# jantonguirao/nvImageCodec

Measured on AMD Instinct MI355X. Metric: images/sec, batched 1920x1080 4:2:0 baseline JPEG decode to interleaved RGB u8, higher is better.
Workload: dtype int32

## Files before the change

### nvimagecodec_amd/csrc/gpu_huffman.hip

```cpp
#include <hip/hip_runtime.h>

#include "gpu_huffman.h"
#include "huffman_gpu_core.h"

namespace hipjpeg {

namespace {

constexpr int kThreads = 256;

constexpr int kRowShift = kSubseqWords == 32 ? 5 : kSubseqWords == 16 ? 4 : kSubseqWords == 64 ? 6 : -1;
static_assert(kRowShift > 0, "subsequences of 512, 1024 or 2048 bits");

#define HJ_LDS __attribute__((address_space(3)))
#define HJ_GLOBAL __attribute__((address_space(1)))
typedef unsigned int u32x4 __attribute__((ext_vector_type(4)));

struct KSlot {
    int16_t* base;
    uint32_t stride_y, stride_x;
};

constexpr int kStagedExtra = 2;
constexpr int kRowWords = kSubseqWords + kStagedExtra;
// ... 312 lines not shown
    const bool markers = im.restart_interval != 0;
    uint32_t before = 0;
    for (uint32_t c = t; c < u.first; c += kThreads) before += drops[im.first_chunk + c];
    before = wg_sum(before, scratch);
    const uint32_t chunk_begin = u.first * kDestuffChunk;
    const uint32_t chunk_len = min((uint32_t)kDestuffChunk, raw_bytes - chunk_begin);
    const uint32_t gout = chunk_begin - before;
    const uint32_t a = gout & 3;

    {
        const uint32_t pieces = (chunk_len + 15) / 16;
        const HJ_GLOBAL u32x4* src = (const HJ_GLOBAL u32x4*)(im.raw + chunk_begin);
        constexpr uint32_t kPiecesPerLane = kDestuffChunk / 16 / kThreads;
        u32x4 v[kPiecesPerLane];
#pragma unroll
        for (uint32_t i = 0; i < kPiecesPerLane; i++) v[i] = src[min(i * kThreads + t, pieces - 1)];
#pragma unroll
        for (uint32_t i = 0; i < kPiecesPerLane; i++) {
            const uint32_t q = i * kThreads + t, g = q * 4 + (q >> 2);
            const u32x4 x = q < pieces ? v[i] : u32x4{0x01010101u, 0x01010101u, 0x01010101u, 0x01010101u};
            buf[g] = x.x;
            buf[g + 1] = x.y;
            buf[g + 2] = x.z;
            buf[g + 3] = x.w;
        }
    }
    const uint32_t before_chunk = chunk_begin > 0 ? im.raw[chunk_begin - 1] : 0u;
    const uint32_t behind_chunk = chunk_len == (uint32_t)kDestuffChunk ? im.raw[chunk_begin + kDestuffChunk] : 0x01u;
    __syncthreads();

    const uint32_t off = chunk_begin + t * 64;
    uint32_t x[16];
    uint32_t gone[4] = {0, 0, 0, 0};
    uint32_t n = 0, len = 0;
    if (off < raw_bytes) {
        len = min(64u, raw_bytes - off);
        const uint32_t pieces = (len + 15) / 16;
        const uint32_t before_lane = t > 0 ? buf[(t - 1) * 17 + 15] >> 24 : before_chunk;
#pragma unroll
        for (uint32_t i = 0; i < 16; i++) x[i] = i < pieces * 4 ? buf[t * 17 + i] : 0x01010101u;
        uint32_t d[16];
        uint32_t prev = before_lane;
#pragma unroll
        for (uint32_t i = 0; i < 16; i++) {
            d[i] = stuffed_zero_mask(x[i], prev);
            prev = x[i] >> 24;
        }
        if (markers) {
            const uint32_t behind = pieces == 4 ? (t < kThreads - 1 ? buf[(t + 1) * 17] & 0xFFu : behind_chunk) : 0x01u;
            prev = before_lane;
#pragma unroll
            for (uint32_t i = 0; i < 16; i++) {
                d[i] |= marker_mask(x[i], prev, i < 15 ? (x[i < 15 ? i + 1 : 15] & 0xFFu) : behind);
                prev = x[i] >> 24;
            }
        }
#pragma unroll
        for (uint32_t i = 0; i < 16; i++) {
            const uint32_t p = __popc(d[i]);
            n += p;
            gone[i / 5] |= p << (6 * (i % 5) + 3);
            const uint32_t m = __builtin_amdgcn_udot4(d[i], 0x08040201u, 0u, false) >> 7;
            x[i] = __builtin_amdgcn_perm(x[i], x[i], squeeze_sel[m]);
        }
    }
    uint32_t incl = n;
    for (int d = 1; d < 64; d <<= 1) {
        const uint32_t v = __shfl_up(incl, d);
        if ((t & 63) >= d) incl += v;
    }
    if ((t & 63) == 63) wave_base[t >> 6] = incl;
    __syncthreads();
    uint32_t excl = incl - n;
    for (int w = 0; w < (t >> 6); w++) excl += wave_base[w];
    const uint32_t chunk_drops = wave_base[0] + wave_base[1] + wave_base[2] + wave_base[3];
    auto padded = [](uint32_t k) { return k + ((k >> 6) << 2); };
    const uint32_t o0 = a + t * 64 - excl, cnt0 = o0 & 3;
    uint32_t slot = o0 >> 2, bits = 8 * cnt0, acc = 0;
    if (len) {
#pragma unroll
        for (uint32_t i = 0; i < 16; i++) {
            const unsigned long long w = (unsigned long long)x[i] << bits;
            const uint32_t p = (gone[i / 5] >> (6 * (i % 5))) & 63u;
            const bool full = bits >= p;
            acc |= (uint32_t)w;
            if (full) buf[slot + (slot >> 4)] = acc;
            acc = full ? (uint32_t)(w >> 32) : acc;
            slot += full ? 1u : 0u;
            bits = (bits - p) & 24u;
        }
    }
    const uint32_t o = slot * 4, cnt = bits / 8;
    __syncthreads();
    {
        const uint32_t from = slot == (o0 >> 2) ? cnt0 : 0u;
#pragma unroll
        for (uint32_t b = 0; b < 3; b++)
            if (b >= from && b < cnt) bytes[padded(o + b)] = (uint8_t)((uint32_t)acc >> (8 * b));
    }
    __syncthreads();
    const uint32_t n_out = chunk_len - chunk_drops;
    uint8_t* dst = const_cast<uint8_t*>(im.stream) + (gout - a);
    const uint32_t first_full = a ? 1 : 0, end_full = (a + n_out) / 4;
    for (uint32_t d = first_full + t; d < end_full; d += kThreads) reinterpret_cast<uint32_t*>(dst)[d] = buf[d + (d >> 4)];
    if (t < 4) {
        if (a && (uint32_t)t >= a && (uint32_t)t < a + n_out) dst[t] = bytes[padded((uint32_t)t)];
        const uint32_t tail = max(end_full, first_full) * 4 + t;
        if (tail >= a && tail < a + n_out && tail >= 4 * first_full) dst[tail] = bytes[padded(tail)];
    }
    if (chunk_begin + chunk_len == raw_bytes) {
        const uint32_t total = raw_bytes - before - chunk_drops;
        const uint32_t padded = ((total + 3) & ~3u) + kStreamSlackBytes;
        uint8_t* s = const_cast<uint8_t*>(im.stream);
        if (total + t < padded) s[total + t] = 0xFF;
        if (t == 0) {
            im.total_bits = total * 8;
            im.num_subseq = (total * 8 + kSubseqBits - 1) / kSubseqBits;
            im.stream_words = padded / 4;
        }
    }
}

__global__ __launch_bounds__(kSyncThreads) void huff_sync_kernel(const HuffImage* __restrict__ images, const HuffUnit* __restrict__ units,
                                                             unsigned long long* __restrict__ states, unsigned long long* __restrict__ incoming,
                                                             unsigned int* __restrict__ counters, int first_pass, int max_rounds,
                                                             uint16_t* __restrict__ tail_tasks, uint32_t* __restrict__ tail_count, uint16_t* records)
{
    __shared__ WgShared sh;
    extern __shared__ uint16_t dyn_pool[];
    HJ_LDS uint16_t* pool = (HJ_LDS uint16_t*)dyn_pool;
    const HuffUnit u = units[blockIdx.x];
    const HuffImage& im = images[u.image];
    const HuffGeom geom = make_geom(im);
    const uint32_t nsub = (geom.total_bits + kSubseqBits - 1) / kSubseqBits;
    if (u.first >= nsub) return;
    unsigned long long* gstate = states + im.first_subseq;
    const int t = threadIdx.x;
    const uint32_t j = u.first - 1 + t;
    const bool owner = t >= 1 && j < nsub;
    const int n_rows = (int)min((uint32_t)kSyncThreads, nsub - u.first + 1);
    unsigned long long in_state = 0;
    if (!first_pass) {
        in_state = u.first ? __hip_atomic_load(&gstate[u.first - 1], __ATOMIC_RELAXED, __HIP_MEMORY_SCOPE_AGENT) & kSyncMask : 0ull;
        if (in_state == incoming[blockIdx.x]) return;
    }
    stage_rows<kSyncThreads>(sh.stream, im, (int)u.first - 1);
    stage_pool<kSyncThreads>(pool, im);
    stage_constants(sh.tsel, nullptr, nullptr, im, false);
    __syncthreads();

    DevEnv env = make_env(sh, pool, u.first, geom);
    const bool rst = im.restart_interval != 0;
    unsigned long long old_global = ~0ull;
    int task = -1;
    const bool recording = !rst;
    if (first_pass) {
        const unsigned long long assumed = (unsigned long long)j * kSubseqBits;
        unsigned long long mine = 0;
        if (owner || (t == 0 && u.first > 0)) {
            const uint32_t bidx0 = boundary0_of(im, j);
            env.set_row(t);
            mine = pack_state(walk_subsequence(rst, false, geom, env, j * kSubseqBits, (j + 1) * kSubseqBits, 0, 0, bidx0, SlotRecorder()));
        }
        sh.end[t] = mine;
        __syncthreads();
        if (owner && ((sh.end[t - 1] & kSyncMask) != assumed || recording)) task = t;
    } else {
        if (owner) old_global = gstate[j];
        sh.end[t] = t == 0 ? in_state : old_global;
        if (t == 1) task = 1;
    }
    int rounds = 0;
    for (int round = 0; round < kSyncThreads + 2; round++) {
        __syncthreads();
        rounds++;
        unsigned long long now = 0;
        bool moved = false;
        if (task >= 0) {
            const SubseqState p = unpack_state(sh.end[task - 1]);
            env.set_row(task);
            const uint32_t jt = u.first - 1 + task;
            const SlotRecorder rec = slot_recorder(records, im, jt);
            const SubseqState st = walk_subsequence(rst, recording, geom, env, p.end_bit, (jt + 1) * kSubseqBits, p.zk & 255, p.zk >> 8, boundary0_of(im, jt), rec);
            if (recording) put_mark(rec, p.end_bit, (jt + 1) * kSubseqBits, geom.total_bits, p.zk & 255, st);
            now = pack_state(st);
            moved = ((now ^ sh.end[task]) & kSyncMask) != 0;
        }
        __syncthreads();
        if (task >= 0) sh.end[task] = now;
        const int pending = compact_tasks(sh, moved && task + 1 < n_rows, task + 1, &task);
        if (pending == 0 || rounds >= max_rounds) {
            if (tail_count) {
                if (t < pending) tail_tasks[(size_t)blockIdx.x * kSyncThreads + t] = (uint16_t)task;
                if (t == 0) tail_count[blockIdx.x] = (uint32_t)pending;
            }
            break;
        }
    }
    __syncthreads();
    if (owner) {
        const unsigned long long mine = sh.end[t];
        if (mine != old_global) {
            __hip_atomic_store(&gstate[j], mine, __ATOMIC_RELAXED, __HIP_MEMORY_SCOPE_AGENT);
            if (t == n_rows - 1 && ((mine ^ old_global) & kSyncMask) != 0) atomicAdd(counters + (first_pass ? 1 : 0), 1u);
        }
    }
    if (t == 0) {
        incoming[blockIdx.x] = first_pass ? (sh.end[0] & kSyncMask) : in_state;
        atomicAdd(counters + (first_pass ? 2 : 4), (unsigned)rounds);
        atomicMax(counters + (first_pass ? 3 : 5), (unsigned)rounds);
    }
}

constexpr int kTailWaves = 4;
constexpr int kTailThreads = 64 * kTailWaves;
#ifndef HJ_TAIL_SLOTS
#define HJ_TAIL_SLOTS 32
#endif
constexpr int kTailSlots = HJ_TAIL_SLOTS;
static_assert(kTailSlots == 32 || kTailSlots == 64, "a power of two, at most one row buffer per lane");
constexpr int kTailRowWords = kSubseqWords + 4;

struct TailWave {
    uint32_t rows[kTailSlots * kTailRowWords];
    uint16_t list[2][kSyncThreads];
    uint32_t count[2];
};
struct TailShared {
    TailWave wave[kTailWaves];
    uint32_t tsel[10];
};

struct TailEnv {
    uint32_t row_base;
    uint32_t word0;
    uint32_t pool;
    const HJ_LDS uint32_t* tsel;
    const uint32_t* boundaries;
    uint32_t num_boundaries;
    __device__ __forceinline__ uint32_t boundary(uint32_t i) const { return load_boundary(boundaries, num_boundaries, i); }
    static constexpr uint32_t kCursorStep = (uint32_t)kTailSlots * 4u;
    __device__ __forceinline__ uint32_t cursor(uint32_t i) const { return row_base + (i - word0) * kCursorStep; }
    __device__ __forceinline__ uint32_t fetch(uint32_t c) const { return *(const HJ_LDS uint32_t*)(uintptr_t)c; }
    __device__ __forceinline__ uint32_t tables(int k) const { return tsel[k]; }
    __device__ __forceinline__ uint32_t lookup1(uint32_t t, uint32_t w) const
    {
        return *(const HJ_LDS uint16_t*)(uintptr_t)(pool + t + ((w >> (31 - kHuffFastBits)) & ((2u << kHuffFastBits) - 2)));
    }
    __device__ __forceinline__ uint32_t lookup2(uint32_t e, uint32_t w) const
    {
        return *(const HJ_LDS uint16_t*)(uintptr_t)(pool + ((e & 0x1FFu) << 7) + ((w >> 15) & ((2u << kHuffSubBits) - 2)));
    }
    __device__ __forceinline__ uint32_t lookup_pair(uint32_t t, uint32_t w) const
    {
        return *(const HJ_LDS uint16_t*)(uintptr_t)(pool + t + 2 * kPairOffset + ((w >> (31 - kHuffFastBits)) & ((2u << kHuffFastBits) - 2)));
    }
};

__device__ __forceinline__ void wave_sync()
{
    __builtin_amdgcn_fence(__ATOMIC_ACQ_REL, "workgroup");
    __builtin_amdgcn_wave_barrier();
}


__device__ __forceinline__ unsigned long long state_in_front(const unsigned long long* states, const HuffImage& im, const HuffUnit u)
{
    return u.first ? __hip_atomic_load(&states[im.first_subseq + u.first - 1], __ATOMIC_RELAXED, __HIP_MEMORY_SCOPE_AGENT) & kSyncMask : 0ull;
}

__device__ __forceinline__ uint32_t uni(uint32_t v) { return (uint32_t)__builtin_amdgcn_readfirstlane((int)v); }
__device__ __forceinline__ uint32_t lane_read(uint32_t v, uint32_t lane) { return (uint32_t)__builtin_amdgcn_readlane((int)v, (int)lane); }

struct CoopWindow {
    uint32_t pool;
    const HJ_LDS uint32_t* tsel;
    const HJ_LDS uint32_t* row;
    uint32_t row_bit0, lane;
    uint32_t edc, eac;
    __device__ __forceinline__ uint32_t tables(uint32_t k) const { return tsel[k]; }
    __device__ __forceinline__ uint32_t entry(uint32_t table, uint32_t w) const
    {
        uint32_t e = *(const HJ_LDS uint16_t*)(uintptr_t)(pool + table + ((w >> (31 - kHuffFastBits)) & ((2u << kHuffFastBits) - 2)));
        if ((e >> 9) == kZadvLong) e = *(const HJ_LDS uint16_t*)(uintptr_t)(pool + ((e & 0x1FFu) << 7) + ((w >> 15) & ((2u << kHuffSubBits) - 2)));
        return e;
    }
    __device__ __forceinline__ void open(uint32_t pos, uint32_t ts)
    {
        const uint32_t b = pos + lane - row_bit0, bit = b & 31u;
        const uint32_t w0 = row[(b >> 5) * kTailSlots], w1 = row[((b >> 5) + 1) * kTailSlots];
        const uint32_t w = bit ? __builtin_amdgcn_alignbit(w0, w1, 32u - bit) : w0;
        edc = entry(ts & 0xFFFFu, w);
        eac = entry(ts >> 16, w);
    }
    __device__ __forceinline__ uint32_t dc(uint32_t rel) const { return lane_read(edc, rel); }
    __device__ __forceinline__ uint32_t ac(uint32_t rel) const { return lane_read(eac, rel); }
};

constexpr int kTailRoundBudget = 192, kRippleRoundBudget = 192;
#ifndef HJ_COOP_CHAINS
#define HJ_COOP_CHAINS 2
#endif
constexpr int kCoopChains = HJ_COOP_CHAINS;

template <bool RIPPLE>
__device__ __forceinline__ void tail_group(TailWave& ws, TailEnv env, HuffImage& im, const HuffUnit u, uint32_t ui, int lane,
                                           unsigned long long* __restrict__ states, unsigned long long* __restrict__ incoming,
                                           unsigned int* __restrict__ counters, const uint16_t* __restrict__ tail_tasks, uint32_t pending,
                                           uint32_t pass_id, uint16_t* records)
{
    const HuffGeom geom = make_geom(im);
    const uint32_t nsub = (geom.total_bits + kSubseqBits - 1) / kSubseqBits;
    if (u.first >= nsub) return;
    unsigned long long* gstate = states + im.first_subseq;
    const int n_rows = (int)min((uint32_t)kSyncThreads, nsub - u.first + 1);
    unsigned long long entering;
    if (RIPPLE) {
        entering = state_in_front(states, im, u);
        if (lane == 0) {
            incoming[ui] = entering;
            ws.list[0][0] = 1;
        }
    } else {
        entering = incoming[ui];
        for (uint32_t i = lane; i < pending; i += 64) ws.list[0][i] = tail_tasks[(size_t)ui * kSyncThreads + i];
    }
    if (lane == 0) ws.count[0] = pending;
    wave_sync();
    const bool rst = im.restart_interval != 0;
    const bool recording = !rst;
    bool out_moved = false;
    const HJ_GLOBAL uint32_t* g = (const HJ_GLOBAL uint32_t*)im.stream;
    const uint32_t gwords = im.stream_words;
    env.row_base = (uint32_t)(uintptr_t)(HJ_LDS uint32_t*)&ws.rows[lane & (kTailSlots - 1)];
    int rounds = 0, cur = 0;
    bool unfinished = false;
    for (int round = 0;; round++) {
        const uint32_t n = ws.count[cur];
        if (n == 0) break;
        if (round >= (RIPPLE ? kRippleRoundBudget : kTailRoundBudget)) {
            unfinished = true;
            break;
        }
        rounds++;
        wave_sync();
        if (lane == 0) ws.count[cur ^ 1] = 0;
        wave_sync();
        if (kCoopChains > 0 && n <= (uint32_t)kCoopChains && !rst) {
            CoopWindow win;
            win.pool = env.pool;
            win.tsel = env.tsel;
            win.row = (const HJ_LDS uint32_t*)&ws.rows[0];
            win.lane = (uint32_t)lane;
            win.edc = win.eac = 0;
            const uint32_t changes = cooperative_table_changes(win, geom.blocks_per_mcu);
            for (uint32_t q = 0; q < n && !unfinished; q++) {
                for (int task = (int)uni(ws.list[cur][q]);; task++) {
                    if (rounds++ >= (RIPPLE ? kRippleRoundBudget : kTailRoundBudget)) {
                        unfinished = true;
                        break;
                    }
                    const unsigned long long before =
                        task == 1 ? entering : __hip_atomic_load(&gstate[u.first - 2 + task], __ATOMIC_RELAXED, __HIP_MEMORY_SCOPE_AGENT);
                    const unsigned long long old = __hip_atomic_load(&gstate[u.first - 1 + task], __ATOMIC_RELAXED, __HIP_MEMORY_SCOPE_AGENT);
                    const uint32_t word0 = (u.first - 1 + task) * kSubseqWords;
                    wave_sync();
                    if (lane < kTailRowWords) {
                        const uint32_t d = word0 + lane;
                        ws.rows[lane * kTailSlots] = d < gwords ? __builtin_bswap32(g[d]) : ~0u;
                    }
                    wave_sync();
                    const SubseqState p = unpack_state(before);
                    win.row_bit0 = word0 * 32u;
                    const uint32_t jt = u.first - 1 + task;
                    const SlotRecorder rec = slot_recorder(records, im, jt);
                    const SubseqState st = cooperative_subsequence(geom, win, changes, p.end_bit, (jt + 1) * kSubseqBits, p.zk & 255u, p.zk >> 8, rec);
                    if (lane == 0) put_mark(rec, p.end_bit, (jt + 1) * kSubseqBits, geom.total_bits, p.zk & 255u, st);
                    const unsigned long long now = pack_state(st);
                    const bool moved = ((now ^ old) & kSyncMask) != 0;
                    if (lane == 0) __hip_atomic_store(&gstate[u.first - 1 + task], now, __ATOMIC_RELAXED, __HIP_MEMORY_SCOPE_AGENT);
                    wave_sync();
                    if (!moved) break;
                    if (task + 1 >= n_rows) {
                        out_moved = true;
                        break;
                    }
                }
            }
            break;
        }
        for (uint32_t base = 0; base < n; base += kTailSlots) {
            const bool busy = lane < kTailSlots && base + lane < n;
            const int task = busy ? (int)ws.list[cur][base + lane] : 1;
            unsigned long long now = 0;
            bool moved = false;
            if (busy) {
                const unsigned long long before =
                    task == 1 ? entering : __hip_atomic_load(&gstate[u.first - 2 + task], __ATOMIC_RELAXED, __HIP_MEMORY_SCOPE_AGENT);
                const unsigned long long old = __hip_atomic_load(&gstate[u.first - 1 + task], __ATOMIC_RELAXED, __HIP_MEMORY_SCOPE_AGENT);
                env.word0 = (u.first - 1 + task) * kSubseqWords;
                HJ_LDS uint32_t* row = (HJ_LDS uint32_t*)(uintptr_t)env.row_base;
#pragma unroll
                for (int i = 0; i < kTailRowWords / 4; i++) {
                    const uint32_t d = env.word0 + 4 * i;
                    const u32x4 x = *(const HJ_GLOBAL u32x4*)(g + min(d, (gwords - 1) & ~3u));
                    const bool ok = d < gwords;
                    row[(4 * i + 0) * kTailSlots] = ok ? __builtin_bswap32(x.x) : ~0u;
                    row[(4 * i + 1) * kTailSlots] = ok ? __builtin_bswap32(x.y) : ~0u;
                    row[(4 * i + 2) * kTailSlots] = ok ? __builtin_bswap32(x.z) : ~0u;
                    row[(4 * i + 3) * kTailSlots] = ok ? __builtin_bswap32(x.w) : ~0u;
                }
                const SubseqState p = unpack_state(before);
                const uint32_t jt = u.first - 1 + task;
                const SlotRecorder rec = slot_recorder(records, im, jt);
                const SubseqState st = walk_subsequence(rst, recording, geom, env, p.end_bit, (jt + 1) * kSubseqBits, p.zk & 255, p.zk >> 8, boundary0_of(im, jt), rec);
                if (recording) put_mark(rec, p.end_bit, (jt + 1) * kSubseqBits, geom.total_bits, p.zk & 255, st);
                now = pack_state(st);
                moved = ((now ^ old) & kSyncMask) != 0;
            }
            wave_sync();
            if (busy) __hip_atomic_store(&gstate[u.first - 1 + task], now, __ATOMIC_RELAXED, __HIP_MEMORY_SCOPE_AGENT);
            out_moved |= busy && moved && task + 1 == n_rows;
            const bool more = busy && moved && task + 1 < n_rows;
            const unsigned long long mask = __ballot(more);
            const uint32_t have = ws.count[cur ^ 1];
            if (more) ws.list[cur ^ 1][have + __popcll(mask & ((1ull << lane) - 1))] = (uint16_t)(task + 1);
            wave_sync();
            if (lane == 0) ws.count[cur ^ 1] = have + (uint32_t)__popcll(mask);
            wave_sync();
        }
        cur ^= 1;
    }
    const bool any_out = __ballot(out_moved) != 0;
    if (lane == 0) {
        atomicAdd(counters + (RIPPLE ? 4 : 6), (unsigned)rounds);
        atomicMax(counters + (RIPPLE ? 5 : 7), (unsigned)rounds);
        if (unfinished) {
            im.gave_up = 1;
        } else if (RIPPLE && any_out) {
            atomicAdd(counters + 0, 1u);
            im.moved_pass = pass_id;
        }
    }
}

template <bool RIPPLE>
__global__ __launch_bounds__(kTailThreads, 5) void huff_tail_kernel(HuffImage* __restrict__ images, const HuffUnit* __restrict__ units, int nunits,
                                                                 unsigned long long* __restrict__ states, unsigned long long* __restrict__ incoming,
                                                                 unsigned int* __restrict__ counters, const uint16_t* __restrict__ tail_tasks,
                                                                 const uint32_t* __restrict__ tail_count, uint32_t pass_id, uint16_t* records)
{
    __shared__ TailShared sh;
    extern __shared__ uint16_t dyn_pool[];
    HJ_LDS uint16_t* pool = (HJ_LDS uint16_t*)dyn_pool;
    const int wave = __builtin_amdgcn_readfirstlane(threadIdx.x >> 6), lane = threadIdx.x & 63;
    const uint32_t ui0 = blockIdx.x * kTailWaves, ui = ui0 + wave;
    const bool valid = ui < (uint32_t)nunits;
    const HuffUnit u = units[valid ? ui : ui0];
    uint32_t todo[kTailWaves];
#pragma unroll
    for (int q = 0; q < kTailWaves; q++) {
        todo[q] = 0;
        if (ui0 + q < (uint32_t)nunits) {
            if (RIPPLE) {
                const HuffUnit uq = units[ui0 + q];
                const HuffImage& iq = images[uq.image];
                const uint32_t nsub = (iq.total_bits + kSubseqBits - 1) / kSubseqBits;
                todo[q] = (uq.first < nsub && iq.gave_up == 0 && state_in_front(states, iq, uq) != incoming[ui0 + q]) ? 1u : 0u;
            } else {
                todo[q] = tail_count[ui0 + q];
            }
        }
    }
    uint32_t pending = 0;
#pragma unroll
    for (int q = 0; q < kTailWaves; q++) pending = q == wave ? todo[q] : pending;
#pragma unroll 1
    for (int s = 0; s < kTailWaves; s++) {
        if (ui0 + s >= (uint32_t)nunits) break;
        const uint32_t image = units[ui0 + s].image;
        if (s > 0 && image == units[ui0 + s - 1].image) continue;
        uint32_t work = 0;
#pragma unroll
        for (int q = 0; q < kTailWaves; q++)
            if (ui0 + q < (uint32_t)nunits && units[ui0 + q].image == image) work |= todo[q];
        if (work == 0) continue;
        HuffImage& im = images[image];
        __syncthreads();
        stage_pool<kTailThreads>(pool, im);
        stage_constants(sh.tsel, nullptr, nullptr, im, false);
        __syncthreads();
        if (valid && u.image == image && pending != 0) {
            TailEnv env;
            env.row_base = 0;
            env.word0 = 0;
            env.pool = (uint32_t)(uintptr_t)pool;
            env.tsel = (const HJ_LDS uint32_t*)sh.tsel;
            env.boundaries = im.boundaries;
            env.num_boundaries = im.num_boundaries;
            tail_group<RIPPLE>(sh.wave[wave], env, im, u, ui, lane, states, incoming, counters, tail_tasks, pending, pass_id, records);
        }
    }
}

constexpr int kCopyCapacity = kHuffOwn * kRecSlots;
constexpr int kSyncWaves = kSyncThreads / 64;
__global__ __launch_bounds__(kSyncThreads) void huff_copy_records_kernel(HuffImage* __restrict__ images, const HuffUnit* __restrict__ units,
                                                                     const unsigned long long* __restrict__ states, uint32_t* __restrict__ first_block,
                                                                     const uint16_t* __restrict__ records, uint32_t* __restrict__ walkers)
{
    __shared__ uint32_t s_pos[kCopyCapacity];
    __shared__ uint32_t s_range[2];
    __shared__ uint32_t s_front[kSyncWaves], s_own[kSyncWaves];
    const HuffUnit u = units[blockIdx.x];
    HuffImage& im = images[u.image];
    const uint32_t nsub = (im.total_bits + kSubseqBits - 1) / kSubseqBits;
    const int t = threadIdx.x;
    const uint32_t j = u.first - 1 + t;
    const bool owner = t != 0 && j < nsub;
    const uint32_t g = im.first_subseq + j;
    const HJ_GLOBAL uint16_t* counts = (const HJ_GLOBAL uint16_t*)(states + im.first_subseq) + 3;
    const uint32_t nfront = min(u.first, nsub);
    uint32_t front = 0;
    constexpr int kBatch = 8;
    for (uint32_t i0 = t; i0 < nfront; i0 += kBatch * kSyncThreads) {
        uint32_t d[kBatch];
#pragma unroll
        for (int k = 0; k < kBatch; k++) {
            const uint32_t i = i0 + k * kSyncThreads;
            d[k] = i < nfront ? counts[(size_t)i * 4] : 0u;
        }
#pragma unroll
        for (int k = 0; k < kBatch; k++) front += d[k];
    }
    const uint32_t own = owner ? counts[(size_t)j * 4] : 0u;
    bool walk = owner;
    uint32_t n = 0, fresh = 0;
    u32x4 v[kRecShorts / 8];
    if (owner && records && im.restart_interval == 0) {
        const HJ_GLOBAL u32x4* src = (const HJ_GLOBAL u32x4*)records + (size_t)g * (kRecShorts / 8);
#pragma unroll
        for (int q = 0; q < kRecShorts / 8; q++) v[q] = src[q];
        const uint32_t mark = v[kRecShorts / 8 - 1].w >> 16;
        if (mark_valid(mark)) {
            walk = false;
            n = mark & (kRecFresh - 1u);
            fresh = mark & kRecFresh;
        }
    }
    for (int off = 32; off > 0; off >>= 1) front += __shfl_xor(front, off);
    uint32_t incl = own;
    for (int d = 1; d < 64; d <<= 1) {
        const uint32_t x = __shfl_up(incl, d);
        if ((t & 63) >= d) incl += x;
    }
    if ((t & 63) == 63) {
        s_front[t >> 6] = front;
        s_own[t >> 6] = incl;
    }
    const int n_walk = __syncthreads_count(walk);
    uint32_t fb = incl - own;
#pragma unroll
    for (int w = 0; w < kSyncWaves; w++) fb += s_front[w] + (w < (t >> 6) ? s_own[w] : 0u);
    if (t == 0) walkers[blockIdx.x] = (uint32_t)n_walk;
    const uint32_t total_blocks = im.total_blocks;
    {
        const uint32_t last_sub = nsub ? nsub - 1 : 0u;
        if (nsub ? j == last_sub && t != 0 : u.first == 0 && t == 0) {
            const uint32_t decoded = fb + own;
            im.decoded_blocks = decoded;
            if (decoded < total_blocks) im.status = 2;
        }
    }
    if (u.first >= nsub) return;
    if (walk) first_block[g] = fb;
    const uint32_t b0 = fb + (fresh ? 0u : 1u);
    HJ_GLOBAL uint32_t* out = (HJ_GLOBAL uint32_t*)im.block_pos;
    const uint32_t bit0 = j * kSubseqBits;
    auto slot = [&](int i) { return bit0 + ((v[i >> 3][(i >> 1) & 3] >> (16 * (i & 1))) & 0xFFFFu); };
    if (n_walk == 0) {
        const int last = (int)min((uint32_t)kSyncThreads, nsub - u.first + 1) - 1;
        if (t == 1) s_range[0] = b0;
        if (t == last) s_range[1] = b0 + n;
        __syncthreads();
        const uint32_t base = s_range[0];
#pragma unroll
        for (int i = 0; i < kRecSlots; i++) {
            const uint32_t at = b0 - base + (uint32_t)i;
            if ((uint32_t)i < n && at < (uint32_t)kCopyCapacity) s_pos[at] = slot(i);
        }
        __syncthreads();
        const uint32_t count = min(s_range[1] - base, (uint32_t)kCopyCapacity);
        for (uint32_t i = t; i < count; i += kSyncThreads)
            if (base + i < total_blocks) out[base + i] = s_pos[i];
    } else if (!walk) {
#pragma unroll
        for (int i = 0; i < kRecSlots; i++)
            if ((uint32_t)i < n && b0 + i < total_blocks) out[b0 + i] = slot(i);
    }
}

__global__ __launch_bounds__(kSyncThreads) void huff_pos_kernel(HuffImage* __restrict__ images, const HuffUnit* __restrict__ units,
                                                            const unsigned long long* __restrict__ states, const uint32_t* __restrict__ first_block,
                                                            const uint16_t* __restrict__ records, const uint32_t* __restrict__ walkers)
{
    __shared__ WgShared sh;
    extern __shared__ uint16_t dyn_pool[];
    HJ_LDS uint16_t* pool = (HJ_LDS uint16_t*)dyn_pool;
    const HuffUnit u = units[blockIdx.x];
    HuffImage& im = images[u.image];
    const HuffGeom geom = make_geom(im);
    const uint32_t nsub = (geom.total_bits + kSubseqBits - 1) / kSubseqBits;
    if (u.first >= nsub) return;
    if (records && walkers[blockIdx.x] == 0) return;
    const int t = threadIdx.x;
    const uint32_t j = u.first - 1 + t;
    const bool rst = im.restart_interval != 0;
    bool walk = t != 0 && j < nsub;
    if (walk && records && !rst) walk = !mark_valid(records[(size_t)(im.first_subseq + j) * kRecShorts + kRecMark]);
    stage_rows<kSyncThreads>(sh.stream, im, (int)u.first - 1);
    stage_pool<kSyncThreads>(pool, im);
    stage_constants(sh.tsel, nullptr, nullptr, im, false);
    __syncthreads();
    if (!walk) return;
    DevEnv env = make_env(sh, pool, u.first, geom);
    env.set_row(t);
    const unsigned long long* st = states + im.first_subseq;
    uint32_t begin = 0;
    int z = 0, k = 0;
    if (j > 0) {
        const SubseqState p = unpack_state(st[j - 1]);
        begin = p.end_bit;
        z = p.zk & 255;
        k = p.zk >> 8;
    }
    HJ_GLOBAL uint32_t* out = (HJ_GLOBAL uint32_t*)im.block_pos;
    const uint32_t total_blocks = im.total_blocks;
    auto rec = [&](uint32_t block, uint32_t pos) {
        if (block < total_blocks) out[block] = pos;
    };
    if (rst) {
        uint32_t fault = 0;
        position_subsequence<true>(geom, env, begin, (j + 1) * kSubseqBits, z, k, first_block[im.first_subseq + j], rec, boundary0_of(im, j), &fault);
        if (fault) im.status = 1;
    } else
        position_subsequence<false>(geom, env, begin, (j + 1) * kSubseqBits, z, k, first_block[im.first_subseq + j], rec);
}

constexpr int kBTeamThreads = kHuffBlocksPerWg;
constexpr int kBTeams = 2;
constexpr int kBThreads = kBTeams * kBTeamThreads;
static_assert((kBTeams & (kBTeams - 1)) == 0, "unit j starts a workgroup when j % kBTeams == 0");
constexpr int kBlockBufBytes = 128;

struct BlockShared {
    KSlot kslot[10];
    uint32_t tsel[10];
    uint32_t zz[16];
    int32_t dc_sum[kBTeams][4];
    uint32_t kcomp[10];
    __attribute__((aligned(128))) uint8_t blocks[kBThreads * kBlockBufBytes];
};
constexpr unsigned kLdsBytesPerCu = 160u * 1024u, kLdsGranule = 1280u, kStandardPoolBytes = 13824u;
constexpr unsigned lds_allocated(unsigned bytes) { return (bytes + kLdsGranule - 1) / kLdsGranule * kLdsGranule; }
static_assert(2 * lds_allocated((unsigned)sizeof(BlockShared) + kStandardPoolBytes) <= kLdsBytesPerCu,
              "two 512-lane workgroups of the block pass per CU (16 waves) with the standard lookup tables");

struct BlockEnv {
    const uint32_t* gstream;
    uint32_t gwords;
    uint32_t pool, buf;
    const HJ_LDS uint32_t* tsel;
    const HJ_LDS KSlot* kslot;
    const HJ_LDS uint8_t* zz;
    static constexpr uint32_t kCursorStep = 1;
    __device__ __forceinline__ uint32_t cursor(uint32_t i) const { return i; }
    __device__ __forceinline__ uint32_t fetch(uint32_t i) const { return word(i); }
    __device__ __forceinline__ uint32_t word(uint32_t i) const
    {
        const uint32_t x = *(const HJ_GLOBAL uint32_t*)((const HJ_GLOBAL char*)gstream + (min(i, gwords - 1) << 2));
        return i < gwords ? __builtin_bswap32(x) : ~0u;
    }
    __device__ __forceinline__ uint32_t tables(int k) const { return tsel[k]; }
    __device__ __forceinline__ uint32_t lookup1(uint32_t t, uint32_t w) const
    {
        return *(const HJ_LDS uint16_t*)(uintptr_t)(pool + t + ((w >> (31 - kHuffFastBits)) & ((2u << kHuffFastBits) - 2)));
    }
    __device__ __forceinline__ uint32_t lookup2(uint32_t e, uint32_t w) const
    {
        return *(const HJ_LDS uint16_t*)(uintptr_t)(pool + ((e & 0x1FFu) << 7) + ((w >> 15) & ((2u << kHuffSubBits) - 2)));
    }
    __device__ __forceinline__ int16_t* block_ptr(int k, uint32_t mx, uint32_t my) const
    {
        const HJ_LDS KSlot* s = kslot + k;
        int16_t* base = s->base;
        const uint32_t sy = s->stride_y, sx = s->stride_x;
        return base + (size_t)(my * sy + mx * sx) * 64;
    }
    __device__ __forceinline__ int zigzag(int z) const { return zz[z]; }
    __device__ __forceinline__ void put(int byte_offset, int value) const { *(HJ_LDS int16_t*)(uintptr_t)(buf ^ (uint32_t)byte_offset) = (int16_t)value; }
};

__global__ __launch_bounds__(kBThreads, 4) void huff_blocks_kernel(HuffImage* __restrict__ images, const HuffUnit* __restrict__ units,
                                                                   uint32_t nunits, int32_t* __restrict__ group_sums)
{
    __shared__ BlockShared sh;
    extern __shared__ uint16_t dyn_pool[];
    HJ_LDS uint16_t* pool = (HJ_LDS uint16_t*)dyn_pool;
    const uint32_t per_team = gridDim.x / (uint32_t)kBTeams;
    const uint32_t unit0 = (blockIdx.x % per_team) * (uint32_t)kBTeams + blockIdx.x / per_team;
    if (unit0 >= nunits) return;
    const HuffUnit u0 = units[unit0];
    if ((u0.first / (uint32_t)kHuffMcusPerWg) % (uint32_t)kBTeams != 0) return;
    HuffImage& im = images[u0.image];
    const HuffGeom geom = make_geom(im);
    const uint32_t bpm = geom.blocks_per_mcu;
    const uint32_t nblocks = min(im.total_blocks, im.decoded_blocks);
    const uint32_t total_mcus = geom.mcus_x * geom.mcus_y;
    const int t = threadIdx.x, team = t / kBTeamThreads, tt = t % kBTeamThreads;
    const uint32_t first = u0.first + (uint32_t)team * kHuffMcusPerWg;
    const bool has_unit = first < total_mcus;
    const uint32_t b_first = first * bpm;
    const uint32_t mcus = has_unit && b_first < nblocks ? min((uint32_t)kHuffMcusPerWg, total_mcus - first) : 0u;
    const uint32_t items = mcus * bpm;
    if (t < 4 * kBTeams) sh.dc_sum[t >> 2][t & 3] = 0;
    if (t >= 32 && t < 42) sh.kcomp[t - 32] = im.k[t - 32].comp & 3;
    stage_pool<kBThreads>(pool, im);
    stage_constants(sh.tsel, sh.kslot, sh.zz, im, true);
    HJ_LDS u32x4* my_buf = (HJ_LDS u32x4*)&sh.blocks[t * kBlockBufBytes];
#pragma unroll
    for (int i = 0; i < kBlockBufBytes / 16; i++) my_buf[i] = u32x4{0u, 0u, 0u, 0u};
    __syncthreads();
    BlockEnv env;
    env.gstream = reinterpret_cast<const uint32_t*>(im.stream);
    env.gwords = im.stream_words;
    env.pool = (uint32_t)(uintptr_t)pool;
    env.buf = (uint32_t)(uintptr_t)(HJ_LDS uint8_t*)sh.blocks + (((uint32_t)t * kBlockBufBytes) | (((uint32_t)t & 7u) << 4));
    env.tsel = (const HJ_LDS uint32_t*)sh.tsel;
    env.kslot = (const HJ_LDS KSlot*)sh.kslot;
    env.zz = (const HJ_LDS uint8_t*)sh.zz;
    uint32_t err = 0;
    static_assert(kBTeamThreads % 64 == 0, "whole waves: lane t flushes the buffers of lanes (t & ~63) ...");
    for (uint32_t base = 0; base < items; base += kBTeamThreads) {
        wave_sync();
        const uint32_t item = base + tt;
        int16_t* dst = nullptr;
        if (item < items) {
            const uint32_t k = item / mcus, mcu = first + (item - k * mcus);
            const uint32_t b = mcu * bpm + k;
            if (b < nblocks) {
                const uint32_t my = mcu / geom.mcus_x, mx = mcu - my * geom.mcus_x;
                dst = env.block_ptr((int)k, mx, my);
                const uint32_t bpos = im.block_pos[b];
                if (geom.interval_blocks != 0 && k == 0 && b != 0 && b % geom.interval_blocks == 0 &&
                    bpos != load_boundary(geom.boundaries, geom.num_boundaries, b / geom.interval_blocks - 1))
                    err = 1;
                const int dc = decode_block(geom, env, bpos, (int)k, &err);
                ((HJ_GLOBAL int16_t*)geom.dc_diff)[b] = (int16_t)dc;
                atomicAdd(&sh.dc_sum[team][sh.kcomp[k]], (int)(int16_t)dc);
            }
        }
        wave_sync();
        const uint32_t dst_lo = (uint32_t)(uintptr_t)dst, dst_hi = (uint32_t)((uintptr_t)dst >> 32);
        const int lane = t & 63, chunk = t & 7;
        int16_t* p[8];
        u32x4 v[8];
#pragma unroll
        for (int i = 0; i < 8; i++) {
            const int src = 8 * i + (lane >> 3);
            const uint32_t lo = (uint32_t)__shfl((int)dst_lo, src, 64), hi = (uint32_t)__shfl((int)dst_hi, src, 64);
            p[i] = (int16_t*)(((uintptr_t)hi << 32) | lo);
        }
#pragma unroll
        for (int i = 0; i < 8; i++) {
            const int blk = (t & ~63) + 8 * i + (lane >> 3);
            v[i] = *(const HJ_LDS u32x4*)&sh.blocks[blk * kBlockBufBytes + ((chunk ^ (blk & 7)) << 4)];
        }
#pragma unroll
        for (int i = 0; i < 8; i++)
            if (p[i]) __builtin_nontemporal_store(v[i], (HJ_GLOBAL u32x4*)p[i] + chunk);
        if (base + kBTeamThreads < items) {
            wave_sync();
#pragma unroll
            for (int i = 0; i < 8; i++) my_buf[i] = u32x4{0u, 0u, 0u, 0u};
        }
    }
    if (err) im.status = 1;
    __syncthreads();
    if (has_unit && tt < 4) group_sums[(size_t)(unit0 + team) * 4 + tt] = sh.dc_sum[team][tt];
}

__global__ __launch_bounds__(kThreads) void huff_dcdiff_kernel(HuffImage* __restrict__ images, const HuffUnit* __restrict__ units,
                                                              int32_t* __restrict__ group_sums)
{
    __shared__ int32_t s_sum[4];
// ... 324 lines not shown
```

Before: 104,000.

## Let tail waves re-enter when the front state changes, and batch their prologue loads

The tail pass now seeds work from the current front state as well as the recorded task list. A wave can re-enter its chain up to a fixed number of times when the preceding subsequence's state changes while it runs. This aims to cut extra ripple passes and kernel relaunches before the chained Huffman synchronisation converges. The kernel prologue also batches the unit, image and state loads across all waves and exits early when no wave has work. The cost is more polling of global state and more complex control flow, and the cooperative branch now loops instead of breaking.

Measured after the change: 106,400 (median of 6 runs). +2.3%, better.

```diff
diff --git a/nvimagecodec_amd/csrc/gpu_huffman.hip b/nvimagecodec_amd/csrc/gpu_huffman.hip
--- a/nvimagecodec_amd/csrc/gpu_huffman.hip
+++ b/nvimagecodec_amd/csrc/gpu_huffman.hip
@@ -638,6 +638,11 @@
 #define HJ_COOP_CHAINS 2
 #endif
 constexpr int kCoopChains = HJ_COOP_CHAINS;
+#ifndef HJ_TAIL_REENTRIES
+#define HJ_TAIL_REENTRIES 4
+#endif
+constexpr uint32_t kTailEnter = 1u << 31;
+constexpr int kTailReentries = HJ_TAIL_REENTRIES;
 
 template <bool RIPPLE>
 __device__ __forceinline__ void tail_group(TailWave& ws, TailEnv env, HuffImage& im, const HuffUnit u, uint32_t ui, int lane,
@@ -650,16 +655,21 @@
     if (u.first >= nsub) return;
     unsigned long long* gstate = states + im.first_subseq;
     const int n_rows = (int)min((uint32_t)kSyncThreads, nsub - u.first + 1);
-    unsigned long long entering;
+    unsigned long long entering = state_in_front(states, im, u);
     if (RIPPLE) {
-        entering = state_in_front(states, im, u);
         if (lane == 0) {
             incoming[ui] = entering;
             ws.list[0][0] = 1;
         }
     } else {
-        entering = incoming[ui];
         for (uint32_t i = lane; i < pending; i += 64) ws.list[0][i] = tail_tasks[(size_t)ui * kSyncThreads + i];
+        if (entering != incoming[ui]) {
+            if (lane == 0) {
+                incoming[ui] = entering;
+                ws.list[0][pending] = 1;
+            }
+            pending++;
+        }
     }
     if (lane == 0) ws.count[0] = pending;
     wave_sync();
@@ -669,12 +679,26 @@
     const HJ_GLOBAL uint32_t* g = (const HJ_GLOBAL uint32_t*)im.stream;
     const uint32_t gwords = im.stream_words;
     env.row_base = (uint32_t)(uintptr_t)(HJ_LDS uint32_t*)&ws.rows[lane & (kTailSlots - 1)];
-    int rounds = 0, cur = 0;
+    int rounds = 0, cur = 0, reentries = 0;
     bool unfinished = false;
-    for (int round = 0;; round++) {
-        const uint32_t n = ws.count[cur];
-        if (n == 0) break;
-        if (round >= (RIPPLE ? kRippleRoundBudget : kTailRoundBudget)) {
+    for (;;) {
+        uint32_t n = ws.count[cur];
+        if (n == 0) {
+            if (RIPPLE || reentries >= kTailReentries || rounds >= kTailRoundBudget) break;
+            const unsigned long long front = state_in_front(states, im, u);
+            if (front == entering) break;
+            reentries++;
+            entering = front;
+            wave_sync();
+            if (lane == 0) {
+                incoming[ui] = entering;
+                ws.list[cur][0] = 1;
+                ws.count[cur] = 1;
+            }
+            wave_sync();
+            n = 1;
+        }
+        if (rounds >= (RIPPLE ? kRippleRoundBudget : kTailRoundBudget)) {
             unfinished = true;
             break;
         }
@@ -723,7 +747,9 @@
                     }
                 }
             }
-            break;
+            if (unfinished) break;
+            cur ^= 1;
+            continue;
         }
         for (uint32_t base = 0; base < n; base += kTailSlots) {
             const bool busy = lane < kTailSlots && base + lane < n;
@@ -794,23 +820,45 @@
     const bool valid = ui < (uint32_t)nunits;
     const HuffUnit u = units[valid ? ui : ui0];
     uint32_t todo[kTailWaves];
-#pragma unroll
-    for (int q = 0; q < kTailWaves; q++) {
-        todo[q] = 0;
-        if (ui0 + q < (uint32_t)nunits) {
-            if (RIPPLE) {
-                const HuffUnit uq = units[ui0 + q];
-                const HuffImage& iq = images[uq.image];
-                const uint32_t nsub = (iq.total_bits + kSubseqBits - 1) / kSubseqBits;
-                todo[q] = (uq.first < nsub && iq.gave_up == 0 && state_in_front(states, iq, uq) != incoming[ui0 + q]) ? 1u : 0u;
-            } else {
-                todo[q] = tail_count[ui0 + q];
-            }
-        }
-    }
+    {
+        HuffUnit uq[kTailWaves];
+        uint32_t bits[kTailWaves], gave[kTailWaves], base[kTailWaves];
+        unsigned long long front[kTailWaves], came[kTailWaves];
+#pragma unroll
+        for (int q = 0; q < kTailWaves; q++) {
+            const uint32_t i = min(ui0 + q, (uint32_t)nunits - 1);
+            uq[q] = units[i];
+            came[q] = incoming[i];
+            todo[q] = RIPPLE ? 0u : tail_count[i];
+        }
+#pragma unroll
+        for (int q = 0; q < kTailWaves; q++) {
+            const HuffImage& iq = images[uq[q].image];
+            bits[q] = iq.total_bits;
+            gave[q] = iq.gave_up;
+            base[q] = iq.first_subseq;
+        }
+#pragma unroll
+        for (int q = 0; q < kTailWaves; q++) {
+            const uint32_t nsub = (bits[q] + kSubseqBits - 1) / kSubseqBits;
+            const bool inside = uq[q].first != 0 && uq[q].first < nsub;
+            front[q] = __hip_atomic_load(&states[inside ? base[q] + uq[q].first - 1 : 0u], __ATOMIC_RELAXED, __HIP_MEMORY_SCOPE_AGENT) & kSyncMask;
+            if (uq[q].first == 0) front[q] = 0;
+            if (uq[q].first >= nsub || gave[q] != 0) front[q] = came[q];
+        }
+#pragma unroll
+        for (int q = 0; q < kTailWaves; q++) {
+            if (front[q] != came[q]) todo[q] |= kTailEnter;
+            if (ui0 + q >= (uint32_t)nunits) todo[q] = 0;
+        }
+        if ((todo[0] | todo[1] | todo[2] | todo[3]) == 0) return;
+    }
+    static_assert(kTailWaves == 4, "the work test above");
     uint32_t pending = 0;
 #pragma unroll
     for (int q = 0; q < kTailWaves; q++) pending = q == wave ? todo[q] : pending;
+    const bool work_here = pending != 0;
+    pending = RIPPLE ? pending >> 31 : pending & ~kTailEnter;
 #pragma unroll 1
     for (int s = 0; s < kTailWaves; s++) {
         if (ui0 + s >= (uint32_t)nunits) break;
@@ -826,7 +874,7 @@
         stage_pool<kTailThreads>(pool, im);
         stage_constants(sh.tsel, nullptr, nullptr, im, false);
         __syncthreads();
-        if (valid && u.image == image && pending != 0) {
+        if (valid && u.image == image && work_here) {
             TailEnv env;
             env.row_base = 0;
             env.word0 = 0;
```
